# alvinwan/neural-backed-decision-trees

Hardware: AMD Instinct MI355X
Metric: images/sec training SoftNBDT WRN28x10 CIFAR10 (higher is better)
Workload: dtype bf16; 1 GPU; WideResNet-28-10 + SoftTreeSupLoss (induced-wrn28_10_cifar10, 10 leaves), CIFAR10-shaped 3x32x32, SGD m=0.9 wd=5e-4; batch_per_gpu=512, global_batch=512, parallelism=dp1

## Files before the change

### include/nbdt_hip.h

```cpp
#ifndef NBDT_HIP_H
#define NBDT_HIP_H

#include <stdint.h>

#ifdef __cplusplus
extern "C" {
#endif

#define NBDT_OK 0
#define NBDT_EINVAL (-1)
#define NBDT_EHIP (-2)
#define NBDT_ENOMEM (-3)

#define NBDT_F32 0
#define NBDT_BF16 1
#define NBDT_F16 2

const char* nbdt_last_error(void);
const char* nbdt_debug_last_igemm(void);
const char* nbdt_debug_last_igemm_full(void);
const char* nbdt_debug_last_wgrad(void);
int nbdt_version(void);
int nbdt_set_deterministic(int32_t on);
int nbdt_get_deterministic(void);
// ... 152 lines not shown
#define NBDT_BN_SLOTS 32
int nbdt_bn_stats(const void* x, int32_t B, int32_t H, int32_t W, int32_t C, float eps,
                  float momentum, float* running_mean, float* running_var, float* scratch,
                  float* save_mean, float* save_rstd, void* stream);
int nbdt_bn_finalize(int32_t B, int32_t H, int32_t W, int32_t C, float eps, float momentum,
                     float* running_mean, float* running_var, const float* bn_partials, float* save_mean,
                     float* save_rstd, void* stream);
int nbdt_bn_apply(const void* x, const float* save_mean, const float* save_rstd, const float* gamma,
                  const float* beta, const void* residual, int32_t relu, int32_t B, int32_t H,
                  int32_t W, int32_t C, void* y, void* stream);
int nbdt_bn_apply_s2d(const void* x, const float* save_mean, const float* save_rstd, const float* gamma,
                      const float* beta, int32_t relu, int32_t B, int32_t H, int32_t W, int32_t C, void* y,
                      void* stream);
int nbdt_bn_bwd_reduce(const void* gy, const void* y, const void* x, const float* save_mean,
                       const float* save_rstd, const float* gamma, const float* beta, int32_t relu,
                       int32_t B, int32_t H, int32_t W, int32_t C, float* scratch, float* dsum,
                       float* dgamma, float* dbeta, void* stream);
int nbdt_bn_bwd_fold(int32_t B, int32_t H, int32_t W, int32_t C, const float* bn_partials, float* dsum,
                     float* dgamma, float* dbeta, void* stream);
int nbdt_bn_bwd_apply(const void* gy, const void* y, const void* x, const float* save_mean,
                      const float* save_rstd, const float* gamma, const float* beta, const float* dsum,
                      const void* gx_add, int32_t relu, int32_t B, int32_t H, int32_t W, int32_t C,
                      void* gx, void* g_resid, void* stream);
int nbdt_bn_bwd_apply_cus(const void* gy, const void* x, const float* save_mean, const float* save_rstd,
                          const float* gamma, const float* beta, const float* dsum, const void* gx_add,
                          int32_t B, int32_t H, int32_t W, int32_t C, void* gx, int32_t cus, void* stream);
int nbdt_bn_bwd_reduce_cus(const void* gy, const void* x, const float* save_mean, const float* save_rstd,
                           const float* gamma, const float* beta, int32_t B, int32_t H, int32_t W, int32_t C,
                           float* scratch, float* dsum, float* dgamma, float* dbeta, int32_t cus, void* stream);
int nbdt_bn_bwd_cus(const void* gy, const void* x, const float* save_mean, const float* save_rstd, const float* gamma,
                    const float* beta, const void* gx_add, int32_t B, int32_t H, int32_t W, int32_t C, float* slots,
                    float* slots_other, float* dsum, float* dgamma, float* dbeta, void* gx, int32_t cus,
                    void* stream);
int nbdt_bn_relu_pool(const void* x, const float* save_mean, const float* save_rstd,
                      const float* gamma, const float* beta, int32_t B, int32_t H, int32_t W,
                      int32_t C, float* pooled, void* stream);
int nbdt_pool_bn_bwd_reduce(const float* gpooled, const void* x, const float* save_mean,
                            const float* save_rstd, const float* gamma, const float* beta,
                            int32_t B, int32_t H, int32_t W, int32_t C, float* scratch, float* dsum,
                            float* dgamma, float* dbeta, void* stream);
int nbdt_pool_bn_bwd_apply(const float* gpooled, const void* x, const float* save_mean,
                           const float* save_rstd, const float* gamma, const float* beta,
                           const float* dsum, int32_t B, int32_t H, int32_t W, int32_t C, void* gx,
                           void* stream);

#define NBDT_ACT_NONE 0
#define NBDT_ACT_RELU 1
#define NBDT_ACT_SWISH 2
int nbdt_bn_act_apply(const void* x, const float* save_mean, const float* save_rstd, const float* gamma,
                      const float* beta, int32_t act, const float* gate, const void* residual, int32_t B,
                      int32_t H, int32_t W, int32_t C, void* y, void* stream);
int nbdt_bn_act_pool(const void* x, const float* save_mean, const float* save_rstd, const float* gamma,
                     const float* beta, int32_t act, const void* mul, float scale, int32_t B, int32_t H,
                     int32_t W, int32_t C, float* out, void* stream);
int nbdt_bn_act_bwd(const void* gu, const float* gate, const float* gpool, const void* x,
                    const float* save_mean, const float* save_rstd, const float* gamma, const float* beta,
                    int32_t act, const void* gx_add, int32_t B, int32_t H, int32_t W, int32_t C,
                    float* scratch, float* dsum, float* dgamma, float* dbeta, void* gx, void* stream);
int nbdt_dwconv_fwd(const void* x, const float* w, int32_t B, int32_t H, int32_t W, int32_t C, int32_t k,
                    int32_t stride, void* y, float* bn_scratch , void* stream);
int nbdt_dwconv_bwd_data(const void* gy, const float* w, int32_t B, int32_t H, int32_t W, int32_t C,
                         int32_t k, int32_t stride, void* gx, void* stream);
int nbdt_dwconv_bwd_data_bn(const void* gy, const float* w, int32_t B, int32_t H, int32_t W, int32_t C, int32_t k,
                            void* gx, const void* bn_x, const float* save_mean, const float* save_rstd,
                            const float* gamma, const float* beta, float* scratch, void* stream);
int nbdt_bn_act_bwd_apply(const void* gu, const void* x, const float* save_mean, const float* save_rstd,
// ... 174 lines not shown
```

### neural-backed-decision-trees_amd/csrc/bn.hip

```cpp
#include "common.h"

using namespace nbdt;

constexpr int kSlots = NBDT_BN_SLOTS;
constexpr int kMaxThreads = 256;

struct Layout {
  int c8, py, threads;
};
static Layout layout_for(int C) {
  Layout l;
  l.c8 = C / 8;
  l.py = kMaxThreads / l.c8;
  if (l.py < 1) l.py = 1;
  l.threads = l.c8 * l.py;
  return l;
}
static int grid_for(const PadGeom& g, const Layout& l, int pixels_per_thread) {
  long long want = ((long long)g.npix + (long long)l.py * pixels_per_thread - 1) / ((long long)l.py * pixels_per_thread);
  if (want < 1) want = 1;
  if (want > 2048) want = 2048;
  return (int)want;
}

// ... 168 lines not shown
      float gg = fg[i];
      if (maskx) gg = (fx[i] * sc[i] + sh[i]) > 0.f ? gg : 0.f;
      else if (RELU) gg = fy[i] > 0.f ? gg : 0.f;
      acc[0][i] += gg;
      acc[1][i] += gg * xh;
    }
  };
  const int step = gridDim.x * PY;
  int p = blockIdx.x * PY + py;
  for (; p + step < g.npix; p += 2 * step) {
    const int o0 = pad_offset(g, p) + cx * 8, o1 = pad_offset(g, p + step) + cx * 8;
    const u32x4_t x0 = *(const u32x4_t*)(x + o0), x1 = *(const u32x4_t*)(x + o1);
    u32x4_t g0 = x0, g1 = x1, y0 = x0, y1 = x1;
    if (!POOL) {
      g0 = *(const u32x4_t*)(gy + o0); g1 = *(const u32x4_t*)(gy + o1);
      if (RELU && !maskx) { y0 = *(const u32x4_t*)(y + o0); y1 = *(const u32x4_t*)(y + o1); }
    }
    one(p, x0, g0, y0);
    one(p + step, x1, g1, y1);
  }
  if (p < g.npix) {
    const int o0 = pad_offset(g, p) + cx * 8;
    const u32x4_t x0 = *(const u32x4_t*)(x + o0);
    u32x4_t g0 = x0, y0 = x0;
    if (!POOL) {
      g0 = *(const u32x4_t*)(gy + o0);
      if (RELU && !maskx) y0 = *(const u32x4_t*)(y + o0);
    }
    one(p, x0, g0, y0);
  }
  block_fold_to_slots<2>(acc, cx, py, c8, PY, g.C, scratch, lds, slot_mask);
}

template <bool RELU, bool POOL, bool HAS_ADD, bool HAS_GRES>
__global__ __launch_bounds__(kMaxThreads) void bn_bwd_apply_kernel(
    const bf16_t* __restrict__ gy, const float* __restrict__ gpooled, const bf16_t* __restrict__ y,
    const bf16_t* __restrict__ x, const float* __restrict__ mean, const float* __restrict__ rstd,
    const float* __restrict__ gamma, const float* __restrict__ beta, const float* __restrict__ dsum,
    const bf16_t* __restrict__ gx_add, PadGeom g, int c8, int PY, bf16_t* __restrict__ gx,
    bf16_t* __restrict__ g_resid) {
  const int cx = threadIdx.x % c8, py = threadIdx.x / c8;
  const float inv_n = 1.f / (float)g.npix;
  const bool maskx = POOL || (RELU && y == nullptr);
  float mu[8], rs[8], sh[8], k0[8], k1[8], sc[8];
#pragma unroll
  for (int i = 0; i < 8; ++i) {
    const int c = cx * 8 + i;
    mu[i] = mean[c];
    rs[i] = rstd[c];
    sc[i] = gamma[c] * rs[i];
    if (maskx) sh[i] = beta[c] - mu[i] * sc[i];
    k0[i] = dsum[c] * inv_n;
    k1[i] = dsum[g.C + c] * inv_n;
  }
  const float inv_hw = 1.f / (float)(g.H * g.W);
  const int hw = g.H * g.W;
  auto one = [&](int p, int o, const u32x4_t vx, const u32x4_t vg, const u32x4_t vy, const u32x4_t va) {
    float fx[8], fg[8], fy[8], fa[8];
    unpack8(vx, fx);
    if (POOL) {
      const int b = p / hw;
#pragma unroll
      for (int i = 0; i < 8; ++i) fg[i] = gpooled[(size_t)b * g.C + cx * 8 + i] * inv_hw;
    } else {
      unpack8(vg, fg);
      if (RELU && !maskx) unpack8(vy, fy);
    }
    if (HAS_ADD) unpack8(va, fa);
    float out[8];
#pragma unroll
    for (int i = 0; i < 8; ++i) {
      const float xh = (fx[i] - mu[i]) * rs[i];
      float gg = fg[i];
      if (maskx) gg = (fx[i] * sc[i] + sh[i]) > 0.f ? gg : 0.f;
      else if (RELU) gg = fy[i] > 0.f ? gg : 0.f;
      fg[i] = gg;
      float v = sc[i] * (gg - k0[i] - xh * k1[i]);
      if (HAS_ADD) v += fa[i];
      out[i] = v;
    }
    *(u32x4_t*)(gx + o) = pack8(out);
    if (HAS_GRES) *(u32x4_t*)(g_resid + o) = pack8(fg);
  };
  auto load = [&](int o, u32x4_t& vx, u32x4_t& vg, u32x4_t& vy, u32x4_t& va) {
    vx = *(const u32x4_t*)(x + o);
    vg = vx; vy = vx; va = vx;
    if (!POOL) {
      vg = *(const u32x4_t*)(gy + o);
      if (RELU && !maskx) vy = *(const u32x4_t*)(y + o);
    }
    if (HAS_ADD) va = *(const u32x4_t*)(gx_add + o);
  };
  const int step = gridDim.x * PY;
  int p = blockIdx.x * PY + py;
  for (; p + step < g.npix; p += 2 * step) {
    const int o0 = pad_offset(g, p) + cx * 8, o1 = pad_offset(g, p + step) + cx * 8;
    u32x4_t x0, g0, y0, a0, x1, g1, y1, a1;
    load(o0, x0, g0, y0, a0);
    load(o1, x1, g1, y1, a1);
    one(p, o0, x0, g0, y0, a0);
    one(p + step, o1, x1, g1, y1, a1);
  }
  if (p < g.npix) {
    const int o0 = pad_offset(g, p) + cx * 8;
    u32x4_t x0, g0, y0, a0;
    load(o0, x0, g0, y0, a0);
    one(p, o0, x0, g0, y0, a0);
  }
}

constexpr int kCusInFlight = 2;
template <bool HAS_ADD, bool FOLD, bool NT>
__global__ __launch_bounds__(1024) void bn_bwd_apply_cus_kernel(
    const bf16_t* __restrict__ gy, const bf16_t* __restrict__ x, const float* __restrict__ mean,
    const float* __restrict__ rstd, const float* __restrict__ gamma, const float* __restrict__ beta,
    const float* __restrict__ dsum, const bf16_t* __restrict__ gx_add, PadGeom g, int c8, int PY,
    bf16_t* __restrict__ gx, const float* __restrict__ slots, float* __restrict__ zero_other,
    float* __restrict__ dsum_out, float* __restrict__ dgamma, float* __restrict__ dbeta) {
  extern __shared__ float fold_lds[];
  if (FOLD) {
    const int C = g.C;
    for (int j = threadIdx.x; j < 2 * C; j += 1024) {
      const int which = j >= C ? 1 : 0, c = j - which * C;
      float s = 0.f;
// ... 436 lines not shown
  rc = slot_target(st, scratch, nblk, 2 * (size_t)C, &t);
  if (rc) return rc;
  if (relu)
    hipLaunchKernelGGL((bn_bwd_reduce_kernel<true, false>), grid, blk, shmem, st, (const bf16_t*)gy, nullptr,
                       (const bf16_t*)y, (const bf16_t*)x, save_mean, save_rstd, gamma, beta, g, l.c8, l.py,
                       t.ptr, t.mask);
  else
    hipLaunchKernelGGL((bn_bwd_reduce_kernel<false, false>), grid, blk, shmem, st, (const bf16_t*)gy, nullptr,
                       (const bf16_t*)y, (const bf16_t*)x, save_mean, save_rstd, gamma, beta, g, l.c8, l.py,
                       t.ptr, t.mask);
  NBDT_LAUNCH_CHECK();
  rc = slot_finish(st, t, nblk, 2 * (size_t)C, scratch);
  if (rc) return rc;
  hipLaunchKernelGGL(bn_bwd_finalize_kernel, dim3((C + 255) / 256), dim3(256), 0, st, scratch, C, dsum, dgamma, dbeta);
  NBDT_LAUNCH_CHECK();
  return NBDT_OK;
}

extern "C" int nbdt_bn_bwd_apply(const void* gy, const void* y, const void* x, const float* save_mean,
                                 const float* save_rstd, const float* gamma, const float* beta, const float* dsum,
                                 const void* gx_add, int32_t relu, int32_t B, int32_t H, int32_t W, int32_t C,
                                 void* gx, void* g_resid, void* stream) {
  NBDT_REQUIRE(gy && x && save_mean && save_rstd && gamma && dsum && gx, "null argument");
  NBDT_REQUIRE(!relu || y || beta, "relu backward needs y, or beta to recompute the mask");
  int rc = check_shape(B, H, W, C);
  if (rc) return rc;
  hipStream_t st = (hipStream_t)stream;
  const PadGeom g = make_geom(B, H, W, C);
  const Layout l = layout_for(C);
  const dim3 grid(grid_for(g, l, 8)), blk(l.threads);
#define NBDT_BA(R, A, G)                                                                                          \
  hipLaunchKernelGGL((bn_bwd_apply_kernel<R, false, A, G>), grid, blk, 0, st, (const bf16_t*)gy, nullptr,          \
                     (const bf16_t*)y, (const bf16_t*)x, save_mean, save_rstd, gamma, beta, dsum,                  \
                     (const bf16_t*)gx_add, g, l.c8, l.py, (bf16_t*)gx, (bf16_t*)g_resid)
  const bool a = gx_add != nullptr, r = g_resid != nullptr;
  if (relu) {
    if (a) { if (r) NBDT_BA(true, true, true); else NBDT_BA(true, true, false); }
    else { if (r) NBDT_BA(true, false, true); else NBDT_BA(true, false, false); }
  } else {
    if (a) { if (r) NBDT_BA(false, true, true); else NBDT_BA(false, true, false); }
    else { if (r) NBDT_BA(false, false, true); else NBDT_BA(false, false, false); }
  }
#undef NBDT_BA
  NBDT_LAUNCH_CHECK();
  return NBDT_OK;
}

extern "C" int nbdt_bn_bwd_apply_cus(const void* gy, const void* x, const float* save_mean, const float* save_rstd,
                                    const float* gamma, const float* beta, const float* dsum, const void* gx_add,
                                    int32_t B, int32_t H, int32_t W, int32_t C, void* gx, int32_t cus,
                                    void* stream) {
  NBDT_REQUIRE(gy && x && save_mean && save_rstd && gamma && beta && dsum && gx, "null argument");
  NBDT_REQUIRE(cus >= 1 && cus <= 256, "cus must be 1..256");
  int rc = check_shape(B, H, W, C);
  if (rc) return rc;
  const PadGeom g = make_geom(B, H, W, C);
  const int c8 = C / 8;
  const int py = 1024 / c8;
  const bool nt = stream_nt((long long)B * g.img * 2);
  constexpr int kForceLds = 96 * 1024;
  static DeviceAttr site;
  if (site.need(kForceLds)) {
    NBDT_ATTR_CHECK(site, hipFuncSetAttribute(reinterpret_cast<const void*>(&bn_bwd_apply_cus_kernel<true, false, false>),
                                              hipFuncAttributeMaxDynamicSharedMemorySize, kForceLds));
    NBDT_ATTR_CHECK(site, hipFuncSetAttribute(reinterpret_cast<const void*>(&bn_bwd_apply_cus_kernel<true, false, true>),
                                              hipFuncAttributeMaxDynamicSharedMemorySize, kForceLds));
    NBDT_ATTR_CHECK(site, hipFuncSetAttribute(reinterpret_cast<const void*>(&bn_bwd_apply_cus_kernel<false, false, false>),
// ... 96 lines not shown
    site.done(kForceLds);
  }
  int blocks = cus;
  const int max_blocks = (g.npix + py - 1) / py;
  if (blocks > max_blocks) blocks = max_blocks;
  SlotTarget t;
  rc = slot_target(st, slots, blocks, 2 * (size_t)C, &t);
  if (rc) return rc;
  { if (nt) hipLaunchKernelGGL((bn_bwd_reduce_cus_kernel<true>), dim3(blocks), dim3(1024), kForceLds, st, (const bf16_t*)gy,
                     (const bf16_t*)x, save_mean, save_rstd, gamma, beta, g, c8, py, t.ptr, t.mask);
    else hipLaunchKernelGGL((bn_bwd_reduce_cus_kernel<false>), dim3(blocks), dim3(1024), kForceLds, st, (const bf16_t*)gy,
                     (const bf16_t*)x, save_mean, save_rstd, gamma, beta, g, c8, py, t.ptr, t.mask); }
  NBDT_LAUNCH_CHECK();
  rc = slot_finish(st, t, blocks, 2 * (size_t)C, slots);
  if (rc) return rc;
  if (gx_add)
    { if (nt) hipLaunchKernelGGL((bn_bwd_apply_cus_kernel<true, true, true>), dim3(blocks), dim3(1024), kForceLds, st, (const bf16_t*)gy,
                       (const bf16_t*)x, save_mean, save_rstd, gamma, beta, nullptr, (const bf16_t*)gx_add, g, c8, py,
                       (bf16_t*)gx, slots, slots_other, dsum, dgamma, dbeta);
      else hipLaunchKernelGGL((bn_bwd_apply_cus_kernel<true, true, false>), dim3(blocks), dim3(1024), kForceLds, st, (const bf16_t*)gy,
                       (const bf16_t*)x, save_mean, save_rstd, gamma, beta, nullptr, (const bf16_t*)gx_add, g, c8, py,
                       (bf16_t*)gx, slots, slots_other, dsum, dgamma, dbeta); }
  else
    { if (nt) hipLaunchKernelGGL((bn_bwd_apply_cus_kernel<false, true, true>), dim3(blocks), dim3(1024), kForceLds, st,
                       (const bf16_t*)gy, (const bf16_t*)x, save_mean, save_rstd, gamma, beta, nullptr, nullptr, g, c8, py,
                       (bf16_t*)gx, slots, slots_other, dsum, dgamma, dbeta);
      else hipLaunchKernelGGL((bn_bwd_apply_cus_kernel<false, true, false>), dim3(blocks), dim3(1024), kForceLds, st,
                       (const bf16_t*)gy, (const bf16_t*)x, save_mean, save_rstd, gamma, beta, nullptr, nullptr, g, c8, py,
                       (bf16_t*)gx, slots, slots_other, dsum, dgamma, dbeta); }
  NBDT_LAUNCH_CHECK();
  return NBDT_OK;
}

extern "C" int nbdt_bn_relu_pool(const void* x, const float* save_mean, const float* save_rstd, const float* gamma,
                                 const float* beta, int32_t B, int32_t H, int32_t W, int32_t C, float* pooled,
                                 void* stream) {
  NBDT_REQUIRE(x && save_mean && save_rstd && gamma && beta && pooled, "null argument");
  int rc = check_shape(B, H, W, C);
  if (rc) return rc;
  const PadGeom g = make_geom(B, H, W, C);
  const int n = B * (C / 8);
  hipLaunchKernelGGL(bn_relu_pool_kernel, dim3((n + 255) / 256), dim3(256), 0, (hipStream_t)stream,
                     (const bf16_t*)x, save_mean, save_rstd, gamma, beta, g, pooled);
  NBDT_LAUNCH_CHECK();
  return NBDT_OK;
}

extern "C" int nbdt_pool_bn_bwd_reduce(const float* gpooled, const void* x, const float* save_mean,
                                       const float* save_rstd, const float* gamma, const float* beta, int32_t B,
                                       int32_t H, int32_t W, int32_t C, float* scratch, float* dsum, float* dgamma,
                                       float* dbeta, void* stream) {
  NBDT_REQUIRE(gpooled && x && save_mean && save_rstd && gamma && beta && scratch && dsum, "null argument");
  int rc = check_shape(B, H, W, C);
  if (rc) return rc;
  hipStream_t st = (hipStream_t)stream;
  const PadGeom g = make_geom(B, H, W, C);
  const Layout l = layout_for(C);
  const size_t shmem = (size_t)l.threads * 16 * sizeof(float);
  const int nblk = grid_for(g, l, 16);
  SlotTarget t;
  rc = slot_target(st, scratch, nblk, 2 * (size_t)C, &t);
  if (rc) return rc;
  hipLaunchKernelGGL((bn_bwd_reduce_kernel<true, true>), dim3(nblk), dim3(l.threads), shmem, st,
                     nullptr, gpooled, nullptr, (const bf16_t*)x, save_mean, save_rstd, gamma, beta, g, l.c8, l.py,
                     t.ptr, t.mask);
  NBDT_LAUNCH_CHECK();
  rc = slot_finish(st, t, nblk, 2 * (size_t)C, scratch);
  if (rc) return rc;
  hipLaunchKernelGGL(bn_bwd_finalize_kernel, dim3((C + 255) / 256), dim3(256), 0, st, scratch, C, dsum, dgamma, dbeta);
  NBDT_LAUNCH_CHECK();
  return NBDT_OK;
}

extern "C" int nbdt_pool_bn_bwd_apply(const float* gpooled, const void* x, const float* save_mean,
                                      const float* save_rstd, const float* gamma, const float* beta,
                                      const float* dsum, int32_t B, int32_t H, int32_t W, int32_t C, void* gx,
                                      void* stream) {
  NBDT_REQUIRE(gpooled && x && save_mean && save_rstd && gamma && beta && dsum && gx, "null argument");
  int rc = check_shape(B, H, W, C);
  if (rc) return rc;
  const PadGeom g = make_geom(B, H, W, C);
  const Layout l = layout_for(C);
  hipLaunchKernelGGL((bn_bwd_apply_kernel<true, true, false, false>), dim3(grid_for(g, l, 8)), dim3(l.threads), 0,
                     (hipStream_t)stream, nullptr, gpooled, nullptr, (const bf16_t*)x, save_mean, save_rstd, gamma,
                     beta, dsum, nullptr, g, l.c8, l.py, (bf16_t*)gx, nullptr);
  NBDT_LAUNCH_CHECK();
  return NBDT_OK;
}
```

### neural-backed-decision-trees_amd/csrc/rules.hip

```cpp
#include "common.h"

#include <algorithm>
#include <vector>

namespace nbdt {
thread_local char g_err[512] = "";
}

using namespace nbdt;

struct nbdt_tree {
  int device;
  int cus;
  int C, N, R, L, root, max_depth;
  int sched_len;
  int32_t* d_all;
  const int32_t *node_off, *slot_off, *slot_cls, *cls_off, *cls_slot, *slot_next;
  const int32_t* sched;
};

struct TreeView {
  int C, N, R, L, root, max_depth, sched_len;
  int tl_ints;
  int staged;
// ... 1244 lines not shown
        lds_count(tot);
        if (iz == yy) lds_count(tot + 1);
        if (hard_cls == yy) lds_count(tot + 2);
        if (want_soft && ip == yy) lds_count(tot + 3);
        lds_count(fed + first_err);
        const int64_t row = yy * t.C;
        if (a.conf_net != nullptr && iz >= 0 && iz < t.C) add_i64(a.conf_net + row + iz, 1);
        if (a.conf_hard != nullptr && hard_cls >= 0 && hard_cls < t.C) add_i64(a.conf_hard + row + hard_cls, 1);
        if (a.conf_soft != nullptr && ip >= 0 && ip < t.C) add_i64(a.conf_soft + row + ip, 1);
      }
      if (want_scores) {
        a.scores[sample * 3] = h_net;
        a.scores[sample * 3 + 1] = top_diff;
        a.scores[sample * 3 + 2] = spread;
      }
    }
    __syncthreads();
  }

  if (a.node_counts != nullptr)
    for (int i = threadIdx.x; i < 5 * t.N; i += (int)blockDim.x)
      if (cnt[i] != 0) add_i64(a.node_counts + i, cnt[i]);
  if (a.totals != nullptr && threadIdx.x < 4 && tot[threadIdx.x] != 0) add_i64(a.totals + threadIdx.x, tot[threadIdx.x]);
  if (a.first_error != nullptr)
    for (int i = threadIdx.x; i <= t.max_depth; i += (int)blockDim.x)
      if (fed[i] != 0) add_i64(a.first_error + i, fed[i]);
  if (a.node_entropy != nullptr)
    for (int i = threadIdx.x; i < 2 * t.N; i += (int)blockDim.x)
      if (ent[i] != 0ull) add_i64(a.node_entropy + i, (long long)ent[i]);
}


extern "C" const char* nbdt_last_error(void) { return nbdt::g_err; }
extern "C" int nbdt_version(void) { return 121; }
extern "C" int nbdt_device_count(void) {
  int n = 0;
  if (hipGetDeviceCount(&n) != hipSuccess) return 0;
  return n;
}

static int pick_tps(int C, int R) { return (C <= 64 && R <= 64) ? 64 : (C <= 512 && R <= 512) ? 256 : 1024; }

static void build_slot_schedule(int R, const int32_t* slot_off, int lanes, std::vector<int32_t>* out, int* len) {
  std::vector<int> order(R);
  for (int s = 0; s < R; ++s) order[s] = s;
  auto length = [&](int s) { return slot_off[s + 1] - slot_off[s]; };
  std::stable_sort(order.begin(), order.end(), [&](int a, int b) { return length(a) > length(b); });
  const int waves = lanes / 64, chunks = (R + 63) / 64;
  std::vector<std::vector<int>> mine(waves);
  std::vector<long> load(waves, 0);
  for (int c = 0; c < chunks; ++c) {
    const int longest = length(order[c * 64]);
    int w = 0;
    for (int i = 1; i < waves; ++i)
      if (load[i] < load[w]) w = i;
    mine[w].push_back(c);
    load[w] += 64 + 8L * longest;
  }
  size_t rows = 0;
  for (auto& m : mine) rows = std::max(rows, m.size());
  const int n = (int)rows * lanes;
  out->assign((size_t)3 * n, -1);
  for (int w = 0; w < waves; ++w)
    for (size_t k = 0; k < mine[w].size(); ++k)
      for (int l = 0; l < 64; ++l) {
        const int i = mine[w][k] * 64 + l;
        if (i >= R) break;
// ... 365 lines not shown
```

### neural-backed-decision-trees_amd/nbdt/_C.py

```python
import ctypes
import os
from ctypes import POINTER, c_char_p, c_float, c_int, c_int32, c_int64, c_void_p

import numpy as np
import torch

_LIBPATH = os.environ.get("NBDT_HIP_LIB") or os.path.join(os.path.dirname(os.path.abspath(__file__)), "_lib",
                                                         "libnbdt_hip.so")
_lib = None

NBDT_F32, NBDT_BF16, NBDT_F16 = 0, 1, 2
NBDT_U8 = 3
NBDT_AUGMENT_MAX_PAD = 32
NBDT_RESIZED_CROP_RATIOS = 4096
NBDT_RESIZED_CROP_ATTEMPTS = 10
NBDT_POLICY_NONE, NBDT_POLICY_TA_WIDE = 0, 1
NBDT_POLICY_OPS = 14
NBDT_POLICY_BINS = 31
_ZTYPE = {torch.float32: NBDT_F32, torch.bfloat16: NBDT_BF16, torch.float16: NBDT_F16}


class NBDTHipError(RuntimeError):
    pass

# ... 86 lines not shown
    "nbdt_hard_tree_loss": (c_int, [c_void_p, _P, c_int, c_int64, c_int64, _P, c_float, c_float, c_float,
                                    _P, _P, _P, _P]),
    "nbdt_soft_tree_loss_ex": (c_int, [c_void_p, _P, c_int, c_int64, c_int64, _P, _P, c_int64, c_float, c_float, c_float,
                                       c_float, _P, _P, _P, _P]),
    "nbdt_hard_tree_loss_ex": (c_int, [c_void_p, _P, c_int, c_int64, c_int64, _P, c_float, c_float, c_float, c_float,
                                       _P, _P, _P, _P]),
    "nbdt_mix_batch": (c_int, [_P, _P, c_int32, c_int32, c_int32, c_float, c_float, c_int32, c_int32, c_int32, c_int32,
                               c_float, c_float, _P, _P, c_int32, _P]),
    "nbdt_node_logits_backward": (c_int, [c_void_p, _P, c_int64, _P, _P]),
    "nbdt_hard_forward": (c_int, [c_void_p, _P, c_int, c_int64, c_int64, _P, _P, _P, _P, _P, _P, _P]),
    "nbdt_node_outputs": (c_int, [c_void_p, _P, c_int, c_int64, c_int64, _P, _P, _P, _P, _P]),
    "nbdt_tree_stats_accumulate": (c_int, [c_void_p, _P, c_int, c_int64, c_int64, _P, _P, _P, _P]),
    "nbdt_conv_igemm": (c_int, [POINTER(ConvDesc), _P, _P, _P, _P, _P]),
    "nbdt_conv_pw": (c_int, [POINTER(ConvDesc), _P, _P, _P, _P, _P]),
    "nbdt_conv_igemm_multi": (c_int, [_P, c_int32, _P, _P, _P, _P]),
    "nbdt_conv_igemm_stats": (c_int, [POINTER(ConvDesc), _P, _P, _P, _P, _P, _P]),
    "nbdt_conv_seg_create": (c_int, [POINTER(ConvSegDesc), POINTER(c_void_p)]),
    "nbdt_conv_seg_destroy": (c_int, [c_void_p]),
    "nbdt_conv_seg_info": (c_int, [c_void_p, _I32P, _I32P, _I32P, _I32P, POINTER(c_int64)]),
    "nbdt_conv_seg_steps": (c_int, [c_void_p, c_int32, _I32P, c_int32, _I32P]),
    "nbdt_conv_seg_tile_weights": (c_int, [c_void_p, POINTER(c_void_p), _P, _P]),
    "nbdt_conv_seg": (c_int, [c_void_p, POINTER(c_void_p), _P, _P, _P, _P, _P]),
    "nbdt_ref_conv_seg": (c_int, [c_void_p, POINTER(c_void_p), POINTER(c_void_p), _P, _P, _P]),
    "nbdt_bn_apply_s2d": (c_int, [_P, _P, _P, _P, _P, c_int32, c_int32, c_int32, c_int32, c_int32, _P, _P]),
    "nbdt_ref_bn_apply_s2d": (c_int, [_P, _P, _P, _P, _P, c_int32, c_int32, c_int32, c_int32, c_int32, _P, _P]),
    "nbdt_bn_finalize": (c_int, [c_int32, c_int32, c_int32, c_int32, c_float, c_float, _P, _P, _P, _P, _P, _P]),
    "nbdt_conv_igemm_bnbwd": (c_int, [POINTER(ConvDesc), _P, _P, _P, _P, _P, _P, _P, _P, _P, _P]),
    "nbdt_conv_igemm_affine": (c_int, [POINTER(ConvDesc), _P, _P, _P, _P, _P, _P, c_int32, _P]),
    "nbdt_bn_bwd_fold": (c_int, [c_int32, c_int32, c_int32, c_int32, _P, _P, _P, _P, _P]),
    "nbdt_bn_bwd_apply_cus": (c_int, [_P, _P, _P, _P, _P, _P, _P, _P, c_int32, c_int32, c_int32, c_int32, _P, c_int32, _P]),
    "nbdt_bn_bwd_reduce_cus": (c_int, [_P, _P, _P, _P, _P, _P, c_int32, c_int32, c_int32, c_int32, _P, _P, _P, _P, c_int32, _P]),
    "nbdt_bn_bwd_cus": (c_int, [_P, _P, _P, _P, _P, _P, _P, c_int32, c_int32, c_int32, c_int32, _P, _P, _P, _P, _P, _P,
                                c_int32, _P]),
    "nbdt_conv_wgrad": (c_int, [POINTER(WgradDesc), _P, _P, _P, _P]),
    "nbdt_ref_conv": (c_int, [POINTER(ConvDesc), _P, _P, _P, _P, _P]),
    "nbdt_ref_wgrad": (c_int, [POINTER(WgradDesc), _P, _P, _P, _P]),
    "nbdt_ref_bn_stats": (c_int, [_P, c_int32, c_int32, c_int32, c_int32, c_float, c_float, _P, _P, _P, _P, _P, _P]),
    "nbdt_ref_bn_apply": (c_int, [_P, _P, _P, _P, _P, _P, c_int32, c_int32, c_int32, c_int32, c_int32, _P, _P]),
    "nbdt_ref_bn_bwd": (c_int, [_P, _P, _P, _P, _P, _P, _P, _P, c_int32, _P, c_int32, c_int32, c_int32, c_int32,
                                c_int32, _P, _P, _P, _P, _P, _P]),
    "nbdt_ref_bn_relu_pool": (c_int, [_P, _P, _P, _P, _P, c_int32, c_int32, c_int32, c_int32, _P, _P]),
    "nbdt_ref_stem_conv": (c_int, [_P, _P, c_int32, c_int32, c_int32, c_int32, c_int32, c_int32, _P, _P]),
    "nbdt_ref_stem_wgrad": (c_int, [_P, _P, c_int32, c_int32, c_int32, c_int32, c_int32, c_int32, _P, _P]),
    "nbdt_ref_bn_act_apply": (c_int, [_P, _P, _P, _P, _P, c_int32, _P, _P, c_int32, c_int32, c_int32, c_int32, _P, _P]),
    "nbdt_ref_bn_act_pool": (c_int, [_P, _P, _P, _P, _P, c_int32, _P, c_float, c_int32, c_int32, c_int32, c_int32, _P,
                                     _P]),
    "nbdt_ref_bn_act_bwd": (c_int, [_P, _P, _P, _P, _P, _P, _P, _P, c_int32, _P, c_int32, c_int32, c_int32, c_int32, _P,
                                    _P, _P, _P, _P]),
    "nbdt_ref_dwconv_fwd": (c_int, [_P, _P, c_int32, c_int32, c_int32, c_int32, c_int32, c_int32, _P, _P]),
    "nbdt_ref_dwconv_bwd_data": (c_int, [_P, _P, c_int32, c_int32, c_int32, c_int32, c_int32, c_int32, _P, _P]),
    "nbdt_ref_dwconv_bwd_weight": (c_int, [_P, _P, c_int32, c_int32, c_int32, c_int32, c_int32, c_int32, _P, _P]),
    "nbdt_weight_prep": (c_int, [_P, c_int32, c_int32, c_int32, _P, _P, _P]),
    "nbdt_weight_prep_batched": (c_int, [_P, _P, c_int32, c_int64, _P, _P]),
    "nbdt_weight_tile_batched": (c_int, [_P, _P, c_int32, c_int64, _P, _P]),
    "nbdt_bn_stats": (c_int, [_P, c_int32, c_int32, c_int32, c_int32, c_float, c_float, _P, _P, _P, _P, _P, _P]),
    "nbdt_bn_apply": (c_int, [_P, _P, _P, _P, _P, _P, c_int32, c_int32, c_int32, c_int32, c_int32, _P, _P]),
    "nbdt_bn_bwd_reduce": (c_int, [_P, _P, _P, _P, _P, _P, _P, c_int32, c_int32, c_int32, c_int32, c_int32,
                                   _P, _P, _P, _P, _P]),
    "nbdt_bn_bwd_apply": (c_int, [_P, _P, _P, _P, _P, _P, _P, _P, _P, c_int32, c_int32, c_int32, c_int32,
                                  c_int32, _P, _P, _P]),
    "nbdt_bn_relu_pool": (c_int, [_P, _P, _P, _P, _P, c_int32, c_int32, c_int32, c_int32, _P, _P]),
    "nbdt_pool_bn_bwd_reduce": (c_int, [_P, _P, _P, _P, _P, _P, c_int32, c_int32, c_int32, c_int32, _P, _P,
                                        _P, _P, _P]),
    "nbdt_pool_bn_bwd_apply": (c_int, [_P, _P, _P, _P, _P, _P, _P, c_int32, c_int32, c_int32, c_int32, _P,
                                       _P]),
    "nbdt_stem_conv": (c_int, [_P, _P, c_int32, c_int32, c_int32, c_int32, c_int32, c_int32, _P, _P]),
    "nbdt_stem_wgrad": (c_int, [_P, _P, c_int32, c_int32, c_int32, c_int32, c_int32, c_int32, _P, _P]),
# ... 316 lines not shown
```

### neural-backed-decision-trees_amd/nbdt/engine.py

```python
import collections
import contextlib
import math

import torch

from nbdt import _C, ops

ALIGN = 8

_SIDE_STREAMS = {}


def side_stream(device):
    dev = torch.device(device)
    key = (dev.type, dev.index if dev.index is not None else torch.cuda.current_device())
    if key not in _SIDE_STREAMS:
        _SIDE_STREAMS[key] = torch.cuda.Stream(device=dev)
    return _SIDE_STREAMS[key]


def _pad32(c):
    return (c + 31) // 32 * 32


# ... 279 lines not shown
    @property
    def gamma(self):
        return self.store.p(self.name + ".weight")

    @property
    def beta(self):
        return self.store.p(self.name + ".bias")

    def stats(self, x, training, fused=False):
        if training:
            self._affine = None
            if fused:
                ops.bn_finalize(x, self.owner.partials(x), self.mean, self.rstd, self.running_mean,
                                self.running_var)
            else:
                ops.bn_stats(x, self.owner.scratch(self.C), self.mean, self.rstd, self.running_mean,
                             self.running_var)
            self.num_batches_tracked += 1
        else:
            self.mean.copy_(self.running_mean)
            torch.rsqrt(self.running_var + ops.BN_EPS, out=self.rstd)

    def apply(self, x, y, relu=True, residual=None):
        ops.bn_apply(x, self.mean, self.rstd, self.gamma, self.beta, y, relu=relu, residual=residual)

    def backward_fused(self, gy, x, gx, partials, gx_add=None, cus=0):
        ops.bn_bwd_fused(gy, x, self.mean, self.rstd, self.gamma, self.beta, partials, self.dsum,
                         self.store.g(self.name + ".weight"), self.store.g(self.name + ".bias"), gx, gx_add=gx_add,
                         cus=cus)

    def backward_cus(self, gy, x, gx, cus, gx_add=None):
        ops.bn_bwd_cus(gy, x, self.mean, self.rstd, self.gamma, self.beta, self.owner.slot_pair(self.C), self.dsum,
                       self.store.g(self.name + ".weight"), self.store.g(self.name + ".bias"), gx, cus, gx_add=gx_add)

    def backward(self, gy, y, x, gx, relu=True, gx_add=None, g_resid=None):
        ops.bn_bwd(gy, y, x, self.mean, self.rstd, self.gamma, self.owner.scratch(self.C), self.dsum,
                   self.store.g(self.name + ".weight"), self.store.g(self.name + ".bias"), gx, relu=relu,
                   gx_add=gx_add, g_resid=g_resid, beta=self.beta)


class _Engine:

    def __init__(self, device, seed):
        self.device = torch.device(device)
        if self.device.type != "cuda":
            raise RuntimeError("the NBDT backbone engine runs on MI355X only (no CPU fallback)")
        self.store = ParamStore(self.device)
        self.gen = torch.Generator().manual_seed(seed)
        self._scratch = None
        self._bufs = {}
        self.convs, self.bns = [], []
        self.training = True
        self.act_dtype = torch.bfloat16
        self.debug_keep = False
        self.debug_share_serial = False
        self.fuse_stats = True
        self.fuse_eval = True
        self.share_bn2_tensors, self.share_bn1_tensors = 5, 6
        self.fuse_bn1_bwd = True
        self._side = None
        self._cu_share = None
        self._share_join = False
        self._share_split = (False, 250.0)
        self._share_calibrated = True
        self.cu_share_report = None
        self._overlap = True
# ... 801 lines not shown
                self._seg_conv1_backward(u, form, g, a1, gt, ga1, g_in)
            else:
                self._conv1_backward(u, form, share, g, a1, gt, ga1, g_in)
            g, h, w = g_in, hi, wi
        ops.stem_wgrad(self._img, g, st.g("features.init_block.weight"), self.stem_c)
        self._end_backward(comm)

    def _backward_form(self):
        two_streams = self._side is not None and self._overlap
        share = self._cu_share is not None and self.fuse_stats and (two_streams or self.debug_share_serial)
        if share and self._share_split[0]:
            return "split", True
        if self.fuse_stats and not (self._cu_share is not None and self._share_split[0]):
            return "fused", share
        return "plain", False

    def _conv2_backward(self, u, form, share, g, a2, t, ga2, gt):
        conv, bn = u["conv2"], u["bn2"]
        B, Hp, Wp, C = gt.shape
        elements = B * (Hp - 2) * (Wp - 2) * C
        if form == "split":
            conv.backward_data(g, ga2)
            n2 = self._share_pair(conv, a2, g, elements, self.share_bn2_tensors, self._split_us(gt))
            bn.backward_cus(ga2, t, gt, n2)
        elif form == "fused":
            if not share:
                conv.backward_weight(a2, g)
            conv.backward_data(g, ga2, bn=bn, bn_x=t, partials=self.partials(t))
            n2 = self._share_pair(conv, a2, g, elements, 3) if share else 0
            bn.backward_fused(ga2, t, gt, self.partials(t), cus=n2)
        else:
            conv.backward_weight(a2, g)
            conv.backward_data(g, ga2)
            bn.backward(ga2, None, t, gt, relu=True)
        if share and self._share_join:
            self.join_side_stream()

    def _conv1_backward(self, u, form, share, g, a1, gt, ga1, g_in):
        conv, bn, x_in = u["conv1"], u["bn1"], u["x_in"]
        B, Hp, Wp, C = ga1.shape
        if u["idconv"] is None and form == "split":
            conv.backward_data(gt, ga1)
            n1 = self._share_pair(conv, a1, gt, B * (Hp - 2) * (Wp - 2) * C, self.share_bn1_tensors, self._split_us(gt))
            bn.backward_cus(ga1, x_in, g_in, n1, gx_add=g)
        elif u["idconv"] is None and form == "fused":
            if not share:
                conv.backward_weight(a1, gt)
            conv.backward_data(gt, ga1, bn=bn, bn_x=x_in, partials=self.partials(x_in))
            n1 = self._share_pair(conv, a1, gt, B * (Hp - 2) * (Wp - 2) * C, 4) if share else 0
            bn.backward_fused(ga1, x_in, g_in, self.partials(x_in), gx_add=g, cus=n1)
        else:
            conv.backward_weight(a1, gt)
            conv.backward_data(gt, ga1)
            if u["idconv"] is not None:
                u["idconv"].backward_weight(a1, g)
                u["idconv"].backward_data(g, ga1, accumulate=True)
                bn.backward(ga1, None, x_in, g_in, relu=True)
            else:
                bn.backward(ga1, None, x_in, g_in, relu=True, gx_add=g)

    def _seg_conv1_backward(self, u, form, g, a1, gt, ga1, g_in):
        c1, ci, bn, x_in, s = u["conv1"], u["idconv"], u["bn1"], u["x_in"], u["stride"]
        B, Hp, Wp, C = ga1.shape
        hi, wi = Hp - 2, Wp - 2
        if form == "split" and s == 2:
            self._seg_dgrad(u, B, hi, wi)([gt, g], ga1)
            gbps, _, lo, hi_cus = self._cu_share
            budget, n1 = ops.plan_cu_share(c1.s2d_plan(B, hi, wi)[1], B * hi * wi * C, self.share_bn2_tensors, gbps,
                                           self._split_us(gt), lo, hi_cus)
            c1.backward_weight_s2d(a1, gt, hi, wi, cu_budget=budget)
            ci.backward_weight_s2d(a1, g, hi, wi)
            bn.backward_cus(ga1, x_in, g_in, n1)
            return
        if s == 2:
            c1.backward_weight_s2d(a1, gt, hi, wi)
            ci.backward_weight_s2d(a1, g, hi, wi)
        else:
            c1.backward_weight(a1, gt)
            ci.backward_weight(a1, g)
        self._seg_dgrad(u, B, hi, wi)([gt, g], ga1)
        bn.backward(ga1, None, x_in, g_in, relu=True)
    def extra_param_views(self, buf):
        return {
            "features.init_block.weight": self.store._view(buf, "features.init_block.weight").permute(0, 3, 1, 2),
            "output.weight": self.store._view(buf, "output.weight"),
            "output.bias": self.store._view(buf, "output.bias"),
        }


class ResNetEngine(_Engine):

    res_share = (47.0, 15.0, 16, 128)

    def __init__(self, num_classes=10, num_blocks=(2, 2, 2, 2), device="cuda", seed=0):
        super().__init__(device, seed)
        self.num_classes = num_classes
        gen = self.gen
        self.stem_c = 64
        self._make_stem()
        self.blocks = []
        cin = 64
        for i, (planes, stride0, n) in enumerate(zip((64, 128, 256, 512), (1, 2, 2, 2), num_blocks)):
            for j in range(n):
                stride = stride0 if j == 0 else 1
                pre, k = f"layer{i + 1}.{j}.", f"l{i + 1}b{j}"
                stages = self._block_stages(pre, cin, planes, stride)
                cout = stages[-1][0].cout_real
                short = stride != 1 or cin != cout
                blk = {
                    "sconv": self.conv(f"{pre}{self.shortcut_name}.0.weight", cin, cout, 1, stride, init=self.conv_init) if short else None,
                    "sbn": self.bn(f"{pre}{self.shortcut_name}.1", cout) if short else None,
                    "cin": cin, "cout": cout, "stride": stride, "key": k,
                }
                head, pairs = [], []
# ... 419 lines not shown
```

### neural-backed-decision-trees_amd/nbdt/ops.py

```python
import ctypes

import torch

from nbdt import _C
from nbdt._C import ConvDesc, WgradDesc, check, lib, ptr

BN_SLOTS = 32
BN_EPS = 1e-5
BN_MOMENTUM = 0.1


def set_deterministic(on):
    check(lib().nbdt_set_deterministic(1 if on else 0))


def is_deterministic():
    return bool(lib().nbdt_get_deterministic())


def set_wgrad_store_epilogue(on):
    check(lib().nbdt_set_wgrad_store_epilogue(1 if on else 0))


def wgrad_store_epilogue():
# ... 292 lines not shown

def bn_bwd_fused(gy, x, mean, rstd, gamma, beta, partials, dsum, dgamma, dbeta, gx, gx_add=None, cus=0):
    _no_ref(x, "bn_bwd_fused: use the split or the unfused schedule")
    B, H, W, C = _dims(x)
    st = stream_ptr(x.device)
    check(lib().nbdt_bn_bwd_fold(B, H, W, C, ptr(partials), ptr(dsum), ptr(dgamma), ptr(dbeta), st))
    if cus > 0:
        check(lib().nbdt_bn_bwd_apply_cus(ptr(gy), ptr(x), ptr(mean), ptr(rstd), ptr(gamma), ptr(beta), ptr(dsum),
                                          ptr(gx_add), B, H, W, C, ptr(gx), int(cus), st))
        return
    check(lib().nbdt_bn_bwd_apply(ptr(gy), None, ptr(x), ptr(mean), ptr(rstd), ptr(gamma), ptr(beta),
                                  ptr(dsum), ptr(gx_add), 1, B, H, W, C, ptr(gx), None, st))


def bn_bwd_cus(gy, x, mean, rstd, gamma, beta, scratch, dsum, dgamma, dbeta, gx, cus, gx_add=None):
    B, H, W, C = _dims(x)
    st = stream_ptr(x.device)
    if _ref(x):
        check(lib().nbdt_ref_bn_bwd(ptr(gy), None, None, ptr(x), ptr(mean), ptr(rstd), ptr(gamma), ptr(beta), 1,
                                    ptr(gx_add), B, H, W, C, 1, ptr(dsum), ptr(dgamma), ptr(dbeta), ptr(gx), None, st))
        return
    if isinstance(scratch, (tuple, list)):
        slots, other = scratch
        check(lib().nbdt_bn_bwd_cus(ptr(gy), ptr(x), ptr(mean), ptr(rstd), ptr(gamma), ptr(beta), ptr(gx_add), B, H, W,
                                    C, ptr(slots), ptr(other), ptr(dsum), ptr(dgamma), ptr(dbeta), ptr(gx), int(cus),
                                    st))
        return
    check(lib().nbdt_bn_bwd_reduce_cus(ptr(gy), ptr(x), ptr(mean), ptr(rstd), ptr(gamma), ptr(beta), B, H, W, C,
                                       ptr(scratch), ptr(dsum), ptr(dgamma), ptr(dbeta), int(cus), st))
    check(lib().nbdt_bn_bwd_apply_cus(ptr(gy), ptr(x), ptr(mean), ptr(rstd), ptr(gamma), ptr(beta), ptr(dsum),
                                      ptr(gx_add), B, H, W, C, ptr(gx), int(cus), st))


def conv_wgrad(desc, x, gy, dw, cu_budget=0):
    desc.cu_budget = int(cu_budget)
    if _ref(x):
        check(lib().nbdt_ref_wgrad(ctypes.byref(desc), ptr(x), ptr(gy), ptr(dw), stream_ptr(x.device)))
        return
    ev = None
    if _timer is not None and _timer.wants("conv_wgrad"):
        flops = desc_flops(desc)
        ev = _timer.bracket("conv_wgrad", flops, x.device)
        ev[0].record()
    check(lib().nbdt_conv_wgrad(ctypes.byref(desc), ptr(x), ptr(gy), ptr(dw), stream_ptr(x.device)))
    if ev is not None:
        ev[1].record()


def conv_wgrad_blocks(desc, cu_budget=0):
    desc.cu_budget = int(cu_budget)
    return int(lib().nbdt_conv_wgrad_blocks(ctypes.byref(desc)))


MI355X_CUS, MI355X_XCDS = 256, 8


def cu_topology_is_mi355x(device):
    props = torch.cuda.get_device_properties(device)
    return props.multi_processor_count == MI355X_CUS and "gfx950" in getattr(props, "gcnArchName", "gfx950")


def plan_cu_share(desc, elements, tensors, gbps_per_cu, target_us, min_cus, max_cus):
    held = (reserved_cus() + MI355X_XCDS - 1) // MI355X_XCDS
    per_xcd = MI355X_CUS // MI355X_XCDS - held
    cus = per_xcd * MI355X_XCDS
    n = int(round(elements * 2 * tensors / (gbps_per_cu * 1e9 * target_us * 1e-6)))
# ... 828 lines not shown
```

Measured before the change: 32390 images/sec.

## Fuse BN backward slot fold into apply kernel with 1024-thread full-device launch

Adds a full-device BN backward path. It runs a 1024-thread reduce into slots, then an apply kernel that folds the slot partials into LDS itself, writes dsum/dgamma/dbeta from block 0 and zeroes the other slot buffer. This removes the separate fold launch and the dsum round trip, and can use non-temporal streaming loads for large tensors. Several residual-block backward calls switch to it. The risk is that every apply block now redundantly re-reads all slots, and the zeroing of the other buffer depends on alternating slot-pair ordering.

New measurement: 32400 images/sec, median of 3. Within noise of the previous version (+0.0%).

```diff
diff --git a/include/nbdt_hip.h b/include/nbdt_hip.h
--- a/include/nbdt_hip.h
+++ b/include/nbdt_hip.h
@@ -208,6 +208,9 @@
                     const float* beta, const void* gx_add, int32_t B, int32_t H, int32_t W, int32_t C, float* slots,
                     float* slots_other, float* dsum, float* dgamma, float* dbeta, void* gx, int32_t cus,
                     void* stream);
+int nbdt_bn_bwd_full(const void* gy, const void* x, const float* save_mean, const float* save_rstd, const float* gamma,
+                     const float* beta, const void* gx_add, int32_t B, int32_t H, int32_t W, int32_t C, float* slots,
+                     float* slots_other, float* dsum, float* dgamma, float* dbeta, void* gx, void* stream);
 int nbdt_bn_relu_pool(const void* x, const float* save_mean, const float* save_rstd,
                       const float* gamma, const float* beta, int32_t B, int32_t H, int32_t W,
                       int32_t C, float* pooled, void* stream);
diff --git a/neural-backed-decision-trees_amd/csrc/bn.hip b/neural-backed-decision-trees_amd/csrc/bn.hip
--- a/neural-backed-decision-trees_amd/csrc/bn.hip
+++ b/neural-backed-decision-trees_amd/csrc/bn.hip
@@ -224,16 +224,36 @@
   block_fold_to_slots<2>(acc, cx, py, c8, PY, g.C, scratch, lds, slot_mask);
 }
 
-template <bool RELU, bool POOL, bool HAS_ADD, bool HAS_GRES>
-__global__ __launch_bounds__(kMaxThreads) void bn_bwd_apply_kernel(
+template <bool RELU, bool POOL, bool HAS_ADD, bool HAS_GRES, bool FOLD = false, bool NT = false>
+__global__ __launch_bounds__(FOLD ? 1024 : kMaxThreads) void bn_bwd_apply_kernel(
     const bf16_t* __restrict__ gy, const float* __restrict__ gpooled, const bf16_t* __restrict__ y,
     const bf16_t* __restrict__ x, const float* __restrict__ mean, const float* __restrict__ rstd,
     const float* __restrict__ gamma, const float* __restrict__ beta, const float* __restrict__ dsum,
     const bf16_t* __restrict__ gx_add, PadGeom g, int c8, int PY, bf16_t* __restrict__ gx,
-    bf16_t* __restrict__ g_resid) {
+    bf16_t* __restrict__ g_resid, const float* __restrict__ slots, float* __restrict__ zero_other,
+    float* __restrict__ dsum_out, float* __restrict__ dgamma, float* __restrict__ dbeta) {
+  extern __shared__ float fold_lds[];
+  if (FOLD) {
+    const int C = g.C;
+    for (int j = threadIdx.x; j < 2 * C; j += blockDim.x) {
+      const int which = j >= C ? 1 : 0, c = j - which * C;
+      float s = 0.f;
+#pragma unroll 8
+      for (int k = 0; k < kSlots; ++k) s += slots[((size_t)k * 2 + which) * C + c];
+      fold_lds[j] = s;
+      if (blockIdx.x == 0) {
+        dsum_out[j] = s;
+        if (which == 0) { if (dbeta) dbeta[c] += s; }
+        else { if (dgamma) dgamma[c] += s; }
+      }
+    }
+    if (blockIdx.x == 0)
+      for (int j = threadIdx.x; j < kSlots * 2 * C; j += blockDim.x) zero_other[j] = 0.f;
+    __syncthreads();
+  }
   const int cx = threadIdx.x % c8, py = threadIdx.x / c8;
   const float inv_n = 1.f / (float)g.npix;
-  const bool maskx = POOL || (RELU && y == nullptr);
+  const bool maskx = POOL || (RELU && (FOLD || y == nullptr));
   float mu[8], rs[8], sh[8], k0[8], k1[8], sc[8];
 #pragma unroll
   for (int i = 0; i < 8; ++i) {
@@ -242,8 +262,8 @@
     rs[i] = rstd[c];
     sc[i] = gamma[c] * rs[i];
     if (maskx) sh[i] = beta[c] - mu[i] * sc[i];
-    k0[i] = dsum[c] * inv_n;
-    k1[i] = dsum[g.C + c] * inv_n;
+    k0[i] = (FOLD ? fold_lds[c] : dsum[c]) * inv_n;
+    k1[i] = (FOLD ? fold_lds[g.C + c] : dsum[g.C + c]) * inv_n;
   }
   const float inv_hw = 1.f / (float)(g.H * g.W);
   const int hw = g.H * g.W;
@@ -275,13 +295,13 @@
     if (HAS_GRES) *(u32x4_t*)(g_resid + o) = pack8(fg);
   };
   auto load = [&](int o, u32x4_t& vx, u32x4_t& vg, u32x4_t& vy, u32x4_t& va) {
-    vx = *(const u32x4_t*)(x + o);
+    vx = ld16_stream<NT>(x + o);
     vg = vx; vy = vx; va = vx;
     if (!POOL) {
-      vg = *(const u32x4_t*)(gy + o);
-      if (RELU && !maskx) vy = *(const u32x4_t*)(y + o);
-    }
-    if (HAS_ADD) va = *(const u32x4_t*)(gx_add + o);
+      vg = ld16_stream<NT>(gy + o);
+      if (RELU && !maskx) vy = ld16_stream<NT>(y + o);
+    }
+    if (HAS_ADD) va = ld16_stream<NT>(gx_add + o);
   };
   const int step = gridDim.x * PY;
   int p = blockIdx.x * PY + py;
@@ -784,7 +804,8 @@
 #define NBDT_BA(R, A, G)                                                                                          \
   hipLaunchKernelGGL((bn_bwd_apply_kernel<R, false, A, G>), grid, blk, 0, st, (const bf16_t*)gy, nullptr,          \
                      (const bf16_t*)y, (const bf16_t*)x, save_mean, save_rstd, gamma, beta, dsum,                  \
-                     (const bf16_t*)gx_add, g, l.c8, l.py, (bf16_t*)gx, (bf16_t*)g_resid)
+                     (const bf16_t*)gx_add, g, l.c8, l.py, (bf16_t*)gx, (bf16_t*)g_resid, nullptr, nullptr, nullptr,  \
+                     nullptr, nullptr)
   const bool a = gx_add != nullptr, r = g_resid != nullptr;
   if (relu) {
     if (a) { if (r) NBDT_BA(true, true, true); else NBDT_BA(true, true, false); }
@@ -947,6 +968,56 @@
   return NBDT_OK;
 }
 
+extern "C" int nbdt_bn_bwd_full(const void* gy, const void* x, const float* save_mean, const float* save_rstd,
+                                const float* gamma, const float* beta, const void* gx_add, int32_t B, int32_t H,
+                                int32_t W, int32_t C, float* slots, float* slots_other, float* dsum, float* dgamma,
+                                float* dbeta, void* gx, void* stream) {
+  NBDT_REQUIRE(gy && x && save_mean && save_rstd && gamma && beta && slots && slots_other && dsum && gx, "null argument");
+  NBDT_REQUIRE(slots != slots_other, "the two slot buffers must be distinct");
+  int rc = check_shape(B, H, W, C);
+  if (rc) return rc;
+  hipStream_t st = (hipStream_t)stream;
+  const PadGeom g = make_geom(B, H, W, C);
+  const bool nt = stream_nt((long long)B * g.img * 2);
+  const int c8 = C / 8, py = 1024 / c8;
+  int blocks = (g.npix + py - 1) / py;
+  if (blocks > 256) blocks = 256;
+  const size_t red_lds = (size_t)py * c8 * 16 * sizeof(float);
+  constexpr int kMaxLds = 96 * 1024;
+  static DeviceAttr site;
+  if (site.need(kMaxLds)) {
+    NBDT_ATTR_CHECK(site, hipFuncSetAttribute(reinterpret_cast<const void*>(&bn_bwd_reduce_cus_kernel<false>),
+                                              hipFuncAttributeMaxDynamicSharedMemorySize, kMaxLds));
+    NBDT_ATTR_CHECK(site, hipFuncSetAttribute(reinterpret_cast<const void*>(&bn_bwd_reduce_cus_kernel<true>),
+                                              hipFuncAttributeMaxDynamicSharedMemorySize, kMaxLds));
+    site.done(kMaxLds);
+  }
+  SlotTarget t;
+  rc = slot_target(st, slots, blocks, 2 * (size_t)C, &t);
+  if (rc) return rc;
+  if (nt)
+    hipLaunchKernelGGL((bn_bwd_reduce_cus_kernel<true>), dim3(blocks), dim3(1024), red_lds, st, (const bf16_t*)gy,
+                       (const bf16_t*)x, save_mean, save_rstd, gamma, beta, g, c8, py, t.ptr, t.mask);
+  else
+    hipLaunchKernelGGL((bn_bwd_reduce_cus_kernel<false>), dim3(blocks), dim3(1024), red_lds, st, (const bf16_t*)gy,
+                       (const bf16_t*)x, save_mean, save_rstd, gamma, beta, g, c8, py, t.ptr, t.mask);
+  NBDT_LAUNCH_CHECK();
+  rc = slot_finish(st, t, blocks, 2 * (size_t)C, slots);
+  if (rc) return rc;
+  const dim3 grid(blocks), blk(c8 * py);
+  const size_t fold_bytes = 2 * (size_t)C * sizeof(float);
+#define NBDT_BF(A, N)                                                                                              \
+  hipLaunchKernelGGL((bn_bwd_apply_kernel<true, false, A, false, true, N>), grid, blk, fold_bytes, st,             \
+                     (const bf16_t*)gy, nullptr, nullptr, (const bf16_t*)x, save_mean, save_rstd, gamma, beta,     \
+                     nullptr, (const bf16_t*)gx_add, g, c8, py, (bf16_t*)gx, nullptr, slots, slots_other, dsum,    \
+                     dgamma, dbeta)
+  if (gx_add) { if (nt) NBDT_BF(true, true); else NBDT_BF(true, false); }
+  else { if (nt) NBDT_BF(false, true); else NBDT_BF(false, false); }
+#undef NBDT_BF
+  NBDT_LAUNCH_CHECK();
+  return NBDT_OK;
+}
+
 extern "C" int nbdt_bn_relu_pool(const void* x, const float* save_mean, const float* save_rstd, const float* gamma,
                                  const float* beta, int32_t B, int32_t H, int32_t W, int32_t C, float* pooled,
                                  void* stream) {
@@ -998,7 +1069,7 @@
   const Layout l = layout_for(C);
   hipLaunchKernelGGL((bn_bwd_apply_kernel<true, true, false, false>), dim3(grid_for(g, l, 8)), dim3(l.threads), 0,
                      (hipStream_t)stream, nullptr, gpooled, nullptr, (const bf16_t*)x, save_mean, save_rstd, gamma,
-                     beta, dsum, nullptr, g, l.c8, l.py, (bf16_t*)gx, nullptr);
-  NBDT_LAUNCH_CHECK();
-  return NBDT_OK;
-}
+                     beta, dsum, nullptr, g, l.c8, l.py, (bf16_t*)gx, nullptr, nullptr, nullptr, nullptr, nullptr, nullptr);
+  NBDT_LAUNCH_CHECK();
+  return NBDT_OK;
+}
diff --git a/neural-backed-decision-trees_amd/csrc/rules.hip b/neural-backed-decision-trees_amd/csrc/rules.hip
--- a/neural-backed-decision-trees_amd/csrc/rules.hip
+++ b/neural-backed-decision-trees_amd/csrc/rules.hip
@@ -1300,7 +1300,7 @@
 
 
 extern "C" const char* nbdt_last_error(void) { return nbdt::g_err; }
-extern "C" int nbdt_version(void) { return 121; }
+extern "C" int nbdt_version(void) { return 122; }
 extern "C" int nbdt_device_count(void) {
   int n = 0;
   if (hipGetDeviceCount(&n) != hipSuccess) return 0;
diff --git a/neural-backed-decision-trees_amd/nbdt/_C.py b/neural-backed-decision-trees_amd/nbdt/_C.py
--- a/neural-backed-decision-trees_amd/nbdt/_C.py
+++ b/neural-backed-decision-trees_amd/nbdt/_C.py
@@ -142,7 +142,8 @@
     "nbdt_bn_bwd_reduce_cus": (c_int, [_P, _P, _P, _P, _P, _P, c_int32, c_int32, c_int32, c_int32, _P, _P, _P, _P, c_int32, _P]),
     "nbdt_bn_bwd_cus": (c_int, [_P, _P, _P, _P, _P, _P, _P, c_int32, c_int32, c_int32, c_int32, _P, _P, _P, _P, _P, _P,
                                 c_int32, _P]),
-    "nbdt_conv_wgrad": (c_int, [POINTER(WgradDesc), _P, _P, _P, _P]),
+    "nbdt_bn_bwd_full": (c_int, [_P, _P, _P, _P, _P, _P, _P, c_int32, c_int32, c_int32, c_int32, _P, _P, _P, _P, _P, _P, _P]),
+    "nbdt_conv_wgrad":(c_int, [POINTER(WgradDesc), _P, _P, _P, _P]),
     "nbdt_ref_conv": (c_int, [POINTER(ConvDesc), _P, _P, _P, _P, _P]),
     "nbdt_ref_wgrad": (c_int, [POINTER(WgradDesc), _P, _P, _P, _P]),
     "nbdt_ref_bn_stats": (c_int, [_P, c_int32, c_int32, c_int32, c_int32, c_float, c_float, _P, _P, _P, _P, _P, _P]),
diff --git a/neural-backed-decision-trees_amd/nbdt/engine.py b/neural-backed-decision-trees_amd/nbdt/engine.py
--- a/neural-backed-decision-trees_amd/nbdt/engine.py
+++ b/neural-backed-decision-trees_amd/nbdt/engine.py
@@ -335,6 +335,10 @@
     def backward_cus(self, gy, x, gx, cus, gx_add=None):
         ops.bn_bwd_cus(gy, x, self.mean, self.rstd, self.gamma, self.beta, self.owner.slot_pair(self.C), self.dsum,
                        self.store.g(self.name + ".weight"), self.store.g(self.name + ".bias"), gx, cus, gx_add=gx_add)
+
+    def backward_full(self, gy, x, gx, gx_add=None):
+        ops.bn_bwd_full(gy, x, self.mean, self.rstd, self.gamma, self.beta, self.owner.slot_pair(self.C), self.dsum,
+                        self.store.g(self.name + ".weight"), self.store.g(self.name + ".bias"), gx, gx_add=gx_add)
 
     def backward(self, gy, y, x, gx, relu=True, gx_add=None, g_resid=None):
         ops.bn_bwd(gy, y, x, self.mean, self.rstd, self.gamma, self.owner.scratch(self.C), self.dsum,
@@ -1202,7 +1206,7 @@
         else:
             conv.backward_weight(a2, g)
             conv.backward_data(g, ga2)
-            bn.backward(ga2, None, t, gt, relu=True)
+            bn.backward_full(ga2, t, gt)
         if share and self._share_join:
             self.join_side_stream()
 
@@ -1225,9 +1229,9 @@
             if u["idconv"] is not None:
                 u["idconv"].backward_weight(a1, g)
                 u["idconv"].backward_data(g, ga1, accumulate=True)
-                bn.backward(ga1, None, x_in, g_in, relu=True)
+                bn.backward_full(ga1, x_in, g_in)
             else:
-                bn.backward(ga1, None, x_in, g_in, relu=True, gx_add=g)
+                bn.backward_full(ga1, x_in, g_in, gx_add=g)
 
     def _seg_conv1_backward(self, u, form, g, a1, gt, ga1, g_in):
         c1, ci, bn, x_in, s = u["conv1"], u["idconv"], u["bn1"], u["x_in"], u["stride"]
@@ -1249,7 +1253,7 @@
             c1.backward_weight(a1, gt)
             ci.backward_weight(a1, g)
         self._seg_dgrad(u, B, hi, wi)([gt, g], ga1)
-        bn.backward(ga1, None, x_in, g_in, relu=True)
+        bn.backward_full(ga1, x_in, g_in)
     def extra_param_views(self, buf):
         return {
             "features.init_block.weight": self.store._view(buf, "features.init_block.weight").permute(0, 3, 1, 2),
diff --git a/neural-backed-decision-trees_amd/nbdt/ops.py b/neural-backed-decision-trees_amd/nbdt/ops.py
--- a/neural-backed-decision-trees_amd/nbdt/ops.py
+++ b/neural-backed-decision-trees_amd/nbdt/ops.py
@@ -348,6 +348,18 @@
                                       ptr(gx_add), B, H, W, C, ptr(gx), int(cus), st))
 
 
+def bn_bwd_full(gy, x, mean, rstd, gamma, beta, pair, dsum, dgamma, dbeta, gx, gx_add=None):
+    B, H, W, C = _dims(x)
+    st = stream_ptr(x.device)
+    if _ref(x):
+        check(lib().nbdt_ref_bn_bwd(ptr(gy), None, None, ptr(x), ptr(mean), ptr(rstd), ptr(gamma), ptr(beta), 1,
+                                    ptr(gx_add), B, H, W, C, 1, ptr(dsum), ptr(dgamma), ptr(dbeta), ptr(gx), None, st))
+        return
+    slots, other = pair
+    check(lib().nbdt_bn_bwd_full(ptr(gy), ptr(x), ptr(mean), ptr(rstd), ptr(gamma), ptr(beta), ptr(gx_add), B, H, W, C,
+                                 ptr(slots), ptr(other), ptr(dsum), ptr(dgamma), ptr(dbeta), ptr(gx), st))
+
+
 def conv_wgrad(desc, x, gy, dw, cu_budget=0):
     desc.cu_budget = int(cu_budget)
     if _ref(x):
```
